# ndefilippis/SWRaytracing

Hardware: AMD Instinct MI355X
Metric: packet-steps/sec @ 512² field, 1e6 packets; 1/2/4/8-GPU scaling (higher is better)
Workload: dtype f64

## Files before the change

### swraytracing_amd/csrc/swrt_api.hip

```cpp
#include <hip/hip_runtime.h>
#include <hip/hip_ext.h>

#include <cmath>
#include <cstdlib>
#include <cstring>
#include <algorithm>
#include <climits>
#include <vector>

#include "../../include/swrt.h"
#include "swrt_bin.hpp"
#include "swrt_fft.hpp"
#include "swrt_kernels.hpp"
#include "swrt_tile.hpp"
#include "swrt_qg.hpp"
#include "swrt_ode23.hpp"
#include "swrt_xka.hpp"
#include "swrt_rsw.hpp"
#include "swrt_spectral.hpp"
#include "swrt_hazard.hpp"
#include "swrt_diag.hpp"
#include "swrt_raydiag.hpp"
#include "swrt_map.hpp"
#include "swrt_kmap.hpp"
// ... 2390 lines not shown
  if (which != 0 && which != 1) return fail(c, SWRT_ERR_ARG, "which must be 0 (current) or 1 (previous)");
  if (which == 1 && !q.has_prev) return fail(c, SWRT_ERR_STATE, "no previous qk before the first step");
  if (layer < 0 || layer >= q.g.nl) return fail(c, SWRT_ERR_ARG, "layer out of range");
  HIPCHK(c, hipSetDevice(c->device));
  const double2* src = (which == 0 ? q.qk.get() : q.qk_prev.get()) + layer * q.nhalf;
  const size_t bytes = sizeof(double2) * q.nhalf;
  if (dst_mode != 0 && dst_mode != 1 && dst_mode != 2) return fail(c, SWRT_ERR_ARG, "dst_mode must be 0, 1 or 2");
  if (dst_mode) {
    const hipStream_t ext = stream ? (hipStream_t)stream : on_qg.saved;
    if (dst_mode == 1) HIPCHK_RC(stream_order(c, ext, c->stream, 0));
    hipLaunchKernelGGL(export_half_kernel, dim3(nblocks(q.nhalf + 1, 256)), dim3(256), 0, c->stream, src, dst,
                       q.nhalf, tail);
    HIPCHK(c, hipGetLastError());
    HIPCHK_RC(stream_order(c, c->stream, ext, 1));
  } else {
    HIPCHK(c, hipMemcpyAsync(dst, src, bytes, hipMemcpyDeviceToHost, c->stream));
    HIPCHK(c, hipStreamSynchronize(c->stream));
    dst[2 * q.nhalf] = tail;
  }
  return SWRT_OK;
  GUARD_END(c)
}

int swrt_snapshot_qk(swrt_ctx* c, int slot, const double* qk, int src_on_device, void* stream, int64_t nx,
                     double L, double K_d2, double shear, double k_scale, int64_t ny_period) {
  int rc = check_slot_args(c, slot, nx);
  if (rc) return rc;
  GUARD_BEGIN_KEEP_CHAIN
  if (!qk) return fail(c, SWRT_ERR_ARG, "qk is NULL");
  if (!is_pow2(nx)) return fail(c, SWRT_ERR_ARG, "nx must be a power of two for the GPU FFT");
  if (!(L > 0)) return fail(c, SWRT_ERR_ARG, "L must be > 0");
  if (ny_period == 0) ny_period = nx;
  if (ny_period % nx) return fail(c, SWRT_ERR_ARG, "ny_period must be a multiple of nx");
  if (c->qg.init && c->qg.g.n != nx) return fail(c, SWRT_ERR_ARG, "nx differs from the QG state's");
  HIPCHK(c, hipSetDevice(c->device));
  const hipStream_t pk = c->stream;
  if (!c->xq.init && !c->qg.init && c->qg_sep) mark_slots_used(c, pk);
  c->xq.init = true;
  OnQGStream on_qg(c);
  const int n = (int)nx, kmax = n / 2 - 1;
  const int64_t nn = nx * nx, nhalf = (int64_t)(2 * kmax + 1) * (kmax + 1);
  if (c->xq.nx != nx) {
    HIPCHK(c, hipStreamSynchronize(c->stream));
    c->xq.nx = 0;
    HIPCHK(c, c->xq.Z.alloc(3 * nn));
    HIPCHK(c, c->xq.T.alloc(3 * nn));
    HIPCHK(c, c->xq.fk.alloc(nhalf));
    c->xq.nx = nx;
  }
  if ((rc = ensure_twiddles(c, n))) return rc;
  if ((rc = qg_slot_acquire(c, slot))) return rc;
  if ((rc = ensure_slot(c, slot, nx))) return rc;
  const hipStream_t ext = stream ? (hipStream_t)stream : pk;
  const double2* fk = (const double2*)qk;
  if (src_on_device) {
    HIPCHK_RC(stream_order(c, ext, c->stream, 0));
  } else {
    HIPCHK(c, hipMemcpyAsync(c->xq.fk.get(), qk, sizeof(double2) * nhalf, hipMemcpyHostToDevice, c->stream));
    HIPCHK(c, hipStreamSynchronize(c->stream));
    fk = c->xq.fk.get();
  }
  if ((rc = fields_from_halfplane(c, slot, fk, n, 1, K_d2, k_scale, shear, 0, c->xq.Z.get(), c->xq.T.get(), n / 2, 1)))
    return rc;
  if (src_on_device) HIPCHK_RC(stream_order(c, c->stream, ext, 1));
  Slot& s = c->slot[slot];
  s.L = L;
  s.ny_period = ny_period;
  return qg_slot_written(c, slot);
  GUARD_END(c)
}

int swrt_swap_slots(swrt_ctx* c, int a, int b) {
  if (!c) return SWRT_ERR_ARG;
  if (a < 0 || a >= SWRT_MAX_SLOTS || b < 0 || b >= SWRT_MAX_SLOTS) return fail(c, SWRT_ERR_ARG, "slot out of range");
  std::swap(c->slot[a], c->slot[b]);
  return SWRT_OK;
}


int swrt_ode23_f1(swrt_ctx* c, double t, double tmax, double f, double Cg, int nslots, double thr, double bump,
                  double* rh_raw_out) {
  if (!c) return SWRT_ERR_ARG;
  GUARD_BEGIN
  HIPCHK_RC(lost_check(c));
  SlotUse slot_use(c, false, kSlots01);
  int rc;
  if ((rc = ode23_f1_queue(c, t, tmax, f, Cg, nslots, thr, bump))) return rc;
  return read_max(c, rh_raw_out);
  GUARD_END(c)
}

int swrt_ode23_attempt(swrt_ctx* c, double t, double h, double tnew, double tmax, double f, double Cg,
                       int nslots, double thr, double bump, double* err_raw_out) {
  if (!c) return SWRT_ERR_ARG;
  GUARD_BEGIN
  HIPCHK_RC(lost_check(c));
  SlotUse slot_use(c, false, kSlots01);
  HIPCHK(c, hipSetDevice(c->device));
  return ode23_attempt(c, t, h, tnew, tmax, f, Cg, nslots, thr, bump, c->o23.dense, err_raw_out);
  GUARD_END(c)
}

int swrt_ode23_accept(swrt_ctx* c) {
  if (!c) return SWRT_ERR_ARG;
  c->s0_dirty = true;
  if (c->in_hook) return fail(c, SWRT_ERR_STATE, "this call may touch the packets: not allowed inside an ode23 hook");
  HIPCHK_RC(lost_check(c));
  HIPCHK_RC(chain_drop(c));
  if (!c->o23.ynx) return fail(c, SWRT_ERR_STATE, "no ode23 step attempted");
  ode23_accept_sets(c);
  return SWRT_OK;
}

int swrt_ode23_set_dense(swrt_ctx* c, int on) {
  if (!c) return SWRT_ERR_ARG;
  c->s0_dirty = true;
  if (on != 0 && on != 1) return fail(c, SWRT_ERR_ARG, "dense must be 0 or 1");
  c->o23.dense = on != 0;
  c->o23.dense_ready = false;
  return SWRT_OK;
}

int swrt_ode23_ntrp(swrt_ctx* c, double t, double tnew, const double* tout, int64_t nout) {
  if (!c) return SWRT_ERR_ARG;
  HOOK_REFUSE
  GUARD_BEGIN_KEEP_CHAIN
  HIPCHK_RC(lost_check(c));
  if (nout < 0) return fail(c, SWRT_ERR_ARG, "nout < 0");
  if (nout > 0 && !tout) return fail(c, SWRT_ERR_ARG, "NULL buffer");
  if (!c->o23.dense_ready)
    return fail(c, SWRT_ERR_STATE,
                "ode23 ntrp: no dense attempt in the stage buffers (swrt_ode23_set_dense 1, then "
                "swrt_ode23_attempt; valid until swrt_ode23_accept or any other packet call)");
  const double tdir = std::copysign(1.0, tnew - t);
  if (!(tnew != t) || !std::isfinite(t) || !std::isfinite(tnew)) return fail(c, SWRT_ERR_ARG, "ode23 ntrp: empty step");
  for (int64_t i = 0; i < nout; ++i)
    if (!(tdir * (tout[i] - t) >= 0 && tdir * (tnew - tout[i]) >= 0))
      return fail(c, SWRT_ERR_ARG, "ode23 ntrp: an output time lies outside the step");
  if (nout == 0) return SWRT_OK;
  HIPCHK(c, hipSetDevice(c->device));
  HIPCHK_RC(ensure_history(c, nout));
  return ode23_ntrp_queue(c, t, tnew, tout, nout);
  GUARD_END(c)
}

int swrt_ode23_run_at(swrt_ctx* c, const double* tspan, int64_t nt, double tmax, double f, double Cg, int nslots,
                      double rtol, double atol, double bump, double* ts_out, int64_t ts_cap, int64_t* nts_out,
                      int64_t* stats3_out) {
  if (!c) return SWRT_ERR_ARG;
  if (!tspan) return fail(c, SWRT_ERR_ARG, "tspan is NULL");
  if (nt < 2) return fail(c, SWRT_ERR_ARG, "tspan needs at least two times");
  if (!ts_out || ts_cap < 1 || !nts_out) return fail(c, SWRT_ERR_ARG, "ts_out / ts_cap / nts_out");
  for (int64_t i = 0; i < nt; ++i)
    if (!std::isfinite(tspan[i])) return fail(c, SWRT_ERR_ARG, "tspan must be finite");
  {
    const double tdir = std::copysign(1.0, tspan[nt - 1] - tspan[0]);
    for (int64_t i = 1; i < nt; ++i)
      if (!(tdir * (tspan[i] - tspan[i - 1]) > 0))
        return fail(c, SWRT_ERR_ARG, "tspan must be strictly increasing or strictly decreasing");
  }
  GUARD_BEGIN
  HIPCHK_RC(lost_check(c));
  SlotUse slot_use(c, false, kSlots01);
  O23Stats st;
  int64_t nts = 0;
  const int rc = ode23_run_at(c, tspan, nt, tmax, f, Cg, nslots, rtol, atol, bump, ts_out, ts_cap, &nts, &st);
  if (rc == kO23BelowHmin) return fail(c, SWRT_ERR_STATE, "ode23: step size below hmin");
  if (rc) return rc;
  *nts_out = nts;
  if (stats3_out) {
    stats3_out[0] = st.steps;
    stats3_out[1] = st.failed;
    stats3_out[2] = st.attempts;
  }
  c->o23.last = st;
  return SWRT_OK;
  GUARD_END(c)
}

int swrt_ode23_chain_next(swrt_ctx* c, int slot_a, int slot_b) {
  if (!c) return SWRT_ERR_ARG;
  if (slot_a < 0 || slot_a >= SWRT_MAX_SLOTS || slot_b < 0 || slot_b >= SWRT_MAX_SLOTS || slot_a == slot_b)
    return fail(c, SWRT_ERR_ARG, "chain slots out of range or equal");
  c->o23.chain.want = true;
  c->o23.chain.sa = slot_a;
  c->o23.chain.sb = slot_b;
  return SWRT_OK;
}

int swrt_ode23_run(swrt_ctx* c, double t0, double tfinal, double tmax, double f, double Cg, int nslots,
                   double rtol, double atol, double bump, double* ts_out, int64_t ts_cap, int64_t* nts_out,
                   int64_t* stats3_out) {
  return swrt_ode23_run_hooked(c, t0, tfinal, tmax, f, Cg, nslots, rtol, atol, bump, ts_out, ts_cap, nts_out,
                               stats3_out, nullptr, nullptr);
}

int swrt_ode23_run_hooked(swrt_ctx* c, double t0, double tfinal, double tmax, double f, double Cg, int nslots,
                          double rtol, double atol, double bump, double* ts_out, int64_t ts_cap, int64_t* nts_out,
                          int64_t* stats3_out, void (*hook)(void*), void* hook_user) {
  return swrt_ode23_run_sharded(c, t0, tfinal, tmax, f, Cg, nslots, rtol, atol, bump, ts_out, ts_cap, nts_out,
                                stats3_out, hook, hook_user, nullptr, nullptr);
}

int swrt_ode23_run_sharded(swrt_ctx* c, double t0, double tfinal, double tmax, double f, double Cg, int nslots,
                           double rtol, double atol, double bump, double* ts_out, int64_t ts_cap, int64_t* nts_out,
                           int64_t* stats3_out, void (*hook)(void*), void* hook_user,
                           int (*reduce)(double*, void*), void* reduce_user) {
  if (!c) return SWRT_ERR_ARG;
  if (!ts_out || ts_cap < 1 || !nts_out) return fail(c, SWRT_ERR_ARG, "ts_out / ts_cap / nts_out");
  if (c->in_hook) return fail(c, SWRT_ERR_STATE, "an ode23 hook may not start another ode23 call");
  GUARD_BEGIN_KEEP_CHAIN
  HIPCHK_RC(lost_check(c));
  SlotUse slot_use(c, false, kSlots01);
  const double rtol_c = std::max(rtol, 100 * 2.220446049250313e-16);
  const double thr = atol / rtol_c;
  const double htspan = std::fabs(tfinal - t0);
  const double hmax = 0.1 * htspan;
  const double c0 = 0.8 * std::pow(rtol_c, 1.0 / 3.0);
  int rc;
  int sl_f1;
  Ode23State::O23Chain& ch = c->o23.chain;
  const bool first_cand = ch.first_q && same_bits(t0, 0.0) && same_bits(tfinal, ch.tfinal) &&
                          same_bits(tmax, ch.tmax) && same_bits(rtol, ch.rtol);
  ch.first_q = false;
  const bool taken = ode23_chain_take(c, t0, tmax, f, Cg, nslots, thr, bump);
  if (!(taken && first_cand)) HIPCHK_RC(chain_join(c));
  if (taken) {
    sl_f1 = ch.dmax_slot;
    ++ch.taken;
  } else {
    if ((rc = ode23_f1_queue(c, t0, tmax, f, Cg, nslots, thr, bump))) return rc;
    sl_f1 = c->o23.dmax_cur;
    c->o23.dmax_cur = (sl_f1 + 1) % 3;
  }
  Ode23Args base;
  if ((rc = ode23_prepare(c, nslots, base, tmax, f, Cg, thr, bump))) return rc;
  const bool dev_first = !reduce && tile_binned(c);
  const bool split = ode23_split_ok(c);
  const bool first_chained = taken && first_cand && dev_first && split == ch.split;
  uint64_t ticket = 0;
  if (first_chained) {
    ticket = ch.first_ticket;
    c->o23.chain_b = false;
    if (split) c->b_pending = 1;
    ++ch.first_taken;
  } else {
    HIPCHK_RC(chain_join(c));
    if (dev_first) {
      HIPCHK_RC(ode23_first_step_queue(c, sl_f1, c0, hmax, htspan, t0, tfinal, split, &ticket));
    } else {
      HIPCHK(c, hipMemcpyAsync(c->o23.hmax.get() + sl_f1, c->o23.dmax.get() + sl_f1, sizeof(unsigned long long),
                               hipMemcpyDeviceToHost, c->stream));
      HIPCHK(c, hipEventRecord(c->o23.ev[sl_f1].get(), c->stream));
    }
    if (split) {
      HIPCHK(c, hipStreamWaitEvent(c->sx[0].get(), c->o23.ev[sl_f1].get(), 0));
      if (c->hz.on) {
        c->hz.record(c->o23.ev[sl_f1].get(), 0);
        c->hz.wait(1, c->o23.ev[sl_f1].get());
      }
      c->b_pending = 1;
    }
  }
  DeviceExec ex(c, base, split, dev_first, sl_f1, hook, hook_user, reduce, reduce_user);
  ex.expect_ticket(ticket);
  if (first_chained)
    ex.adopt_first(ch.first_slot, ch.first_wg);
  else if (dev_first && (rc = ex.queue_first()))
    return rc;
  O23Stats st;
  int64_t nts = 0;
  rc = ode23_control(ex, t0, tfinal, rtol, atol, ts_out, ts_cap, &nts, &st);
  if (rc == kO23BelowHmin) return fail(c, SWRT_ERR_STATE, "ode23: step size below hmin");
  if (rc) return rc;
  if ((rc = ode23_chain_queue(c, tmax, f, Cg, nslots, thr, bump, rtol, reduce == nullptr))) return rc;
  *nts_out = nts;
  if (stats3_out) {
    stats3_out[0] = st.steps;
    stats3_out[1] = st.failed;
    stats3_out[2] = st.attempts;
  }
  c->o23.last = st;
  c->o23.first_taken += st.first_taken;
  c->o23.guesses_taken += st.guesses_taken[0] + st.guesses_taken[1] + st.guesses_taken[2];
  c->o23.split_runs += split ? 1 : 0;
  return SWRT_OK;
  GUARD_END(c)
}

#ifdef SWRT_PHASE_TIMING
int swrt_debug_phases(unsigned long long* out, int ntiles, int clear) {
  if (hipDeviceSynchronize() != hipSuccess) return SWRT_ERR_HIP;
  const size_t bytes = (size_t)ntiles * 8 * sizeof(unsigned long long);
  if (out && hipMemcpyFromSymbol(out, HIP_SYMBOL(swrt::swrt_phase_dbg), bytes, 0, hipMemcpyDeviceToHost) != hipSuccess)
    return SWRT_ERR_HIP;
  if (clear) {
    static unsigned long long zeros[16384 * 8];
    if (hipMemcpyToSymbol(HIP_SYMBOL(swrt::swrt_phase_dbg), zeros, sizeof(zeros), 0,
                          hipMemcpyHostToDevice) != hipSuccess)
      return SWRT_ERR_HIP;
  }
  return SWRT_OK;
}
#endif

}
```

### swraytracing_amd/csrc/swrt_tile.hpp

```cpp
#pragma once
#include <hip/hip_runtime.h>
#include <stdint.h>

#include "swrt_kernels.hpp"

namespace swrt {

struct TileArgs {
  StepArgs s;
  double* x_out;
  double* k_out;
  int* perm_out;
  const int* starts;
  const int* order;
  int ntx;
  int* next_keys;
  int* next_counts;
  int sort_cells;
  const int* src;
  double sort_lead;
  TileShare sh;
  int ivmode;
  int nint;
  const double* ivn[kMaxIntervals + 1];
  double ivdt[kMaxIntervals];
  StageArgs stg;
};

__device__ __forceinline__ auto tile_args_again() {
  auto* p = (const __attribute__((address_space(4))) TileArgs*)__builtin_amdgcn_kernarg_segment_ptr();
  asm volatile("" : "+s"(p));
  return p;
}

__device__ __forceinline__ const double* iv_nodes(const TileArgs& ta, int i) {
  const double* p = ta.ivn[0];
#pragma unroll
  for (int j = 1; j <= kMaxIntervals; ++j)
    if (i == j) p = ta.ivn[j];
  return p;
}
__device__ __forceinline__ double iv_dt(const TileArgs& ta, int i) {
  double d = ta.ivdt[0];
#pragma unroll
  for (int j = 1; j < kMaxIntervals; ++j)
    if (i == j) d = ta.ivdt[j];
  return d;
}

__device__ __forceinline__ int wg_work_range(const int* starts, const int* order, int64_t n, const TileShare& sh,
                                             int& pbeg, int& pend) {
  int tile = share_slot(sh, (int)blockIdx.x);
  if (order != nullptr) tile = order[tile];
  const int nn = (int)n;
  pbeg = min(max(starts[tile], 0), nn);
  pend = min(max(starts[tile + 1], pbeg), nn);
  return tile;
}
__device__ __forceinline__ int wg_work_range(const int* starts, int64_t n, int& pbeg, int& pend) {
  TileShare sh;
  sh.ntiles = (int)gridDim.x;
  return wg_work_range(starts, nullptr, n, sh, pbeg, pend);
}

__device__ __forceinline__ int wg_work(const TileArgs& ta, int& pbeg, int& pend) {
  return wg_work_range(ta.starts, ta.order, ta.s.n, ta.sh, pbeg, pend);
}

__device__ __forceinline__ int ring_diff(int a, int b, int n) {
  int d = a - b;
  if (d >= n / 2) d -= n;
  if (d < -n / 2) d += n;
  return d;
}

__device__ __forceinline__ int b128_lane_rank(int lane) {
  const int h = lane & 32, t = lane & 31;
  int k;
  if (t < 4) k = t;
  else if (t < 12) k = 16 + (t - 4);
  else if (t < 16) k = 4 + (t - 12);
  else if (t < 20) k = 24 + (t - 16);
  else if (t < 28) k = 8 + (t - 20);
  else k = t;
  return h + k;
}

template <bool TWO>
struct Tap6 {
  double2 a0, a1, a2, b0, b1, b2;
};
template <bool TWO, int WN>
__device__ __forceinline__ void tap6_read(const double2* p, int e, Tap6<TWO>& t) {
  t.a0 = p[0 * WN + e];
  t.a1 = p[1 * WN + e];
  t.a2 = p[2 * WN + e];
  if constexpr (TWO) {
    t.b0 = p[3 * WN + e];
    t.b1 = p[4 * WN + e];
    t.b2 = p[5 * WN + e];
  }
}
template <bool TWO, int W, int WN>
__device__ __forceinline__ void gather6_lds(const double2* lds, int node0, const Stencil& s,
                                            double o0[kRec], double o1[kRec]) {
#pragma unroll
  for (int f = 0; f < kRec; ++f) { o0[f] = -0.0; o1[f] = -0.0; }
  const double2* p = lds + node0;
  double wx[kNT], wy[kNT];
#pragma unroll
  for (int q = 0; q < kNT; ++q) {
    wx[q] = s.wx[q];
    wy[q] = s.wy[q];
    asm volatile("" : "+v"(wx[q]));
    asm volatile("" : "+v"(wy[q]));
  }
  if constexpr (TWO) {
#pragma unroll
    for (int i = 0; i < kNT; ++i) {
#pragma unroll
      for (int j = 0; j < kNT; ++j) {
        const int e = i * W + j;
        const double wij = wx[i] * wy[j];
        const double2 a0 = p[0 * WN + e], a1 = p[1 * WN + e], a2 = p[2 * WN + e];
        o0[0] = o0[0] + wij * a0.x; o0[1] = o0[1] + wij * a0.y;
        o0[2] = o0[2] + wij * a1.x; o0[3] = o0[3] + wij * a1.y;
        o0[4] = o0[4] + wij * a2.x; o0[5] = o0[5] + wij * a2.y;
        const double2 b0 = p[3 * WN + e], b1 = p[4 * WN + e], b2 = p[5 * WN + e];
        o1[0] = o1[0] + wij * b0.x; o1[1] = o1[1] + wij * b0.y;
        o1[2] = o1[2] + wij * b1.x; o1[3] = o1[3] + wij * b1.y;
        o1[4] = o1[4] + wij * b2.x; o1[5] = o1[5] + wij * b2.y;
      }
    }
    return;
  }
  Tap6<TWO> cur, nxt;
  tap6_read<TWO, WN>(p, 0, cur);
#pragma unroll
  for (int t = 0; t < kNT * kNT; ++t) {
    const int i = t / kNT, j = t % kNT;
    if (t + 1 < kNT * kNT) tap6_read<TWO, WN>(p, ((t + 1) / kNT) * W + (t + 1) % kNT, nxt);
    if constexpr (!TWO) __builtin_amdgcn_sched_barrier(0);
    const double wij = wx[i] * wy[j];
    o0[0] = o0[0] + wij * cur.a0.x; o0[1] = o0[1] + wij * cur.a0.y;
    o0[2] = o0[2] + wij * cur.a1.x; o0[3] = o0[3] + wij * cur.a1.y;
    o0[4] = o0[4] + wij * cur.a2.x; o0[5] = o0[5] + wij * cur.a2.y;
    if constexpr (TWO) {
      o1[0] = o1[0] + wij * cur.b0.x; o1[1] = o1[1] + wij * cur.b0.y;
      o1[2] = o1[2] + wij * cur.b1.x; o1[3] = o1[3] + wij * cur.b1.y;
      o1[4] = o1[4] + wij * cur.b2.x; o1[5] = o1[5] + wij * cur.b2.y;
    }
    if constexpr (!TWO) __builtin_amdgcn_sched_barrier(0);
    if (t + 1 < kNT * kNT) cur = nxt;
  }
}

template <bool TWO>
struct Tap5 {
  double2 a0, a1, c, b0, b1;
};
template <bool TWO, int WN>
__device__ __forceinline__ void tap5_read(const double2* p, int e, Tap5<TWO>& t) {
  t.a0 = p[0 * WN + e];
  t.a1 = p[1 * WN + e];
  if constexpr (TWO) {
    t.c = p[2 * WN + e];
    t.b0 = p[3 * WN + e];
    t.b1 = p[4 * WN + e];
  } else {
    t.c.x = reinterpret_cast<const double*>(p + 2 * WN + e)[0];
  }
}
template <bool TWO, int W, int WN, bool FMA = false, int PF = 1>
__device__ __forceinline__ void gather5_lds(const double2* lds, int node0, const Stencil& s,
                                            double o0[kRec], double o1[kRec]) {
  static_assert(PF >= 1 && PF <= 4, "prefetch depth");
  constexpr int NTAP = kNT * kNT;
#pragma unroll
  for (int f = 0; f < 5; ++f) { o0[f] = -0.0; o1[f] = -0.0; }
  const double2* p = lds + node0;
  double wx[kNT], wy[kNT];
#pragma unroll
  for (int q = 0; q < kNT; ++q) {
    wx[q] = s.wx[q];
    wy[q] = s.wy[q];
    asm volatile("" : "+v"(wx[q]));
    asm volatile("" : "+v"(wy[q]));
  }
  Tap5<TWO> ring[PF + 1];
#pragma unroll
  for (int t = 0; t < PF; ++t) tap5_read<TWO, WN>(p, (t / kNT) * W + t % kNT, ring[t]);
#pragma unroll
  for (int t = 0; t < NTAP; ++t) {
    const int i = t / kNT, j = t % kNT;
    if (t + PF < NTAP) tap5_read<TWO, WN>(p, ((t + PF) / kNT) * W + (t + PF) % kNT, ring[(t + PF) % (PF + 1)]);
    __builtin_amdgcn_sched_barrier(0);
    const Tap5<TWO>& cur = ring[t % (PF + 1)];
    const double wij = wx[i] * wy[j];
    o0[0] = madd<FMA>(o0[0], wij, cur.a0.x); o0[1] = madd<FMA>(o0[1], wij, cur.a0.y);
    o0[2] = madd<FMA>(o0[2], wij, cur.a1.x); o0[3] = madd<FMA>(o0[3], wij, cur.a1.y);
    o0[4] = madd<FMA>(o0[4], wij, cur.c.x);
    if constexpr (TWO) {
      o1[0] = madd<FMA>(o1[0], wij, cur.b0.x); o1[1] = madd<FMA>(o1[1], wij, cur.b0.y);
      o1[2] = madd<FMA>(o1[2], wij, cur.b1.x); o1[3] = madd<FMA>(o1[3], wij, cur.b1.y);
      o1[4] = madd<FMA>(o1[4], wij, cur.c.y);
    }
    __builtin_amdgcn_sched_barrier(0);
  }
  o0[5] = -o0[2];
  o1[5] = -o1[2];
}

template <bool TWO, int W, int WN>
__device__ __forceinline__ void gather2_lds(const double2* lds, int node0, const Stencil& s, double o0[2],
                                            double o1[2]) {
  constexpr int NTAP = kNT * kNT;
  o0[0] = o0[1] = -0.0;
  o1[0] = o1[1] = -0.0;
  const double2* p = lds + node0;
  double wx[kNT], wy[kNT];
#pragma unroll
  for (int q = 0; q < kNT; ++q) {
    wx[q] = s.wx[q];
    wy[q] = s.wy[q];
    asm volatile("" : "+v"(wx[q]));
    asm volatile("" : "+v"(wy[q]));
  }
  double2 ra[2], rb[2];
  ra[0] = p[0];
  if constexpr (TWO) rb[0] = p[3 * WN];
#pragma unroll
  for (int t = 0; t < NTAP; ++t) {
    const int i = t / kNT, j = t % kNT;
    if (t + 1 < NTAP) {
      const int e = ((t + 1) / kNT) * W + (t + 1) % kNT;
      ra[(t + 1) & 1] = p[e];
      if constexpr (TWO) rb[(t + 1) & 1] = p[3 * WN + e];
    }
    __builtin_amdgcn_sched_barrier(0);
    const double wij = wx[i] * wy[j];
    o0[0] = o0[0] + wij * ra[t & 1].x; o0[1] = o0[1] + wij * ra[t & 1].y;
    if constexpr (TWO) {
      o1[0] = o1[0] + wij * rb[t & 1].x; o1[1] = o1[1] + wij * rb[t & 1].y;
    }
    __builtin_amdgcn_sched_barrier(0);
  }
}

template <bool TWO, int WN, bool V5>
__device__ __forceinline__ void stage_record(const double2* s0, const double2* s1, int d, double2* win) {
  if constexpr (V5 && TWO) {
    const double2 a0 = s0[0], a1 = s0[1], a2 = s0[2], b0 = s1[0], b1 = s1[1], b2 = s1[2];
    win[0 * WN + d] = a0;
    win[1 * WN + d] = a1;
    win[2 * WN + d] = make_double2(a2.x, b2.x);
    win[3 * WN + d] = b0;
    win[4 * WN + d] = b1;
  } else if constexpr (TWO) {
    const double2 a0 = s0[0], a1 = s0[1], a2 = s0[2], b0 = s1[0], b1 = s1[1], b2 = s1[2];
    win[0 * WN + d] = a0;
    win[1 * WN + d] = a1;
    win[2 * WN + d] = a2;
    win[3 * WN + d] = b0;
    win[4 * WN + d] = b1;
    win[5 * WN + d] = b2;
  } else {
    const double2 a0 = s0[0], a1 = s0[1], a2 = s0[2];
    win[0 * WN + d] = a0;
    win[1 * WN + d] = a1;
    win[2 * WN + d] = a2;
  }
}
template <bool TWO, int T, int M, int NT, int WS = T + 5 + 2 * M, bool V5 = false>
__device__ __forceinline__ void stage_window_regs(const FieldView& f0, const FieldView& f1, int ox, int oy,
                                                  double2* win) {
  constexpr int W = T + 5 + 2 * M;
  constexpr int WN = W * WS;
  constexpr int CW = W <= 32 ? 32 : (W <= 64 ? 64 : 128);
  constexpr int RP = NT / CW;
  static_assert(W <= CW && NT % CW == 0, "window rows per workgroup pass");
  const int nx = f0.nx, npad = f0.npad;
  const int wj = (int)threadIdx.x % CW;
  int wi = (int)threadIdx.x / CW;
  if (wj >= W) return;
  const char* n0 = reinterpret_cast<const char*>(f0.nodes);
  const char* n1 = reinterpret_cast<const char*>(f1.nodes);
  constexpr unsigned kRecBytes = kRec * sizeof(double);
  if (nx >= W && (uint64_t)npad * (uint64_t)npad * kRecBytes < (1ull << 32)) {
    int gy = oy - M - 2 + wj;
    gy += gy < 0 ? nx : 0;
    gy -= gy >= nx ? nx : 0;
    const unsigned col = (unsigned)(gy + kPadLo) * kRecBytes;
    const unsigned rowb = (unsigned)npad * kRecBytes;
    for (int d = wi * WS + wj; wi < W; wi += RP, d += RP * WS) {
      int gx = ox - M - 2 + wi;
      gx += gx < 0 ? nx : 0;
      gx -= gx >= nx ? nx : 0;
      const unsigned off = (unsigned)(gx + kPadLo) * rowb + col;
      stage_record<TWO, WN, V5>(reinterpret_cast<const double2*>(n0 + off),
                                reinterpret_cast<const double2*>(n1 + off), d, win);
    }
  } else {
    int gy = (oy - M - 2 + wj) % nx; gy += gy < 0 ? nx : 0;
    for (; wi < W; wi += RP) {
      int gx = (ox - M - 2 + wi) % nx; gx += gx < 0 ? nx : 0;
      const size_t off = ((size_t)(gx + kPadLo) * npad + (gy + kPadLo)) * kRecBytes;
      stage_record<TWO, WN, V5>(reinterpret_cast<const double2*>(n0 + off),
                                reinterpret_cast<const double2*>(n1 + off), wi * WS + wj, win);
    }
  }
}

#ifdef SWRT_PHASE_TIMING
__device__ unsigned long long swrt_phase_dbg[16384 * 8];
#define SWRT_STAMP(slot)                                                            \
  do {                                                                              \
    if (tid == 0) swrt_phase_dbg[blockIdx.x * 8 + (slot)] = __builtin_amdgcn_s_memrealtime(); \
  } while (0)
#else
#define SWRT_STAMP(slot) \
  do {                   \
  } while (0)
#endif

template <int T, int NT, int NB>
__device__ __forceinline__ void sort_batch_by_cell(int b0, int nb, bool first_batch, int tile, int* hist,
                                                   int* kr, int* order) {
  const auto* g = tile_args_again();
  int tid = threadIdx.x;
  asm volatile("" : "+v"(tid));
  const int nx = g->s.f0.nx;
  const int tx = (int)((unsigned)tile / (unsigned)g->ntx), ty = tile - tx * g->ntx;
  const int ox = tx * T, oy = ty * T;
  const int64_t n = g->s.n;
  const double* xin = g->s.x;
  const double* kin = g->s.k;
  const int* srcp = g->src;
  const double sort_lead = g->sort_lead, gH = g->s.gH, f2 = g->s.f2, inv_dx = g->s.f0.inv_dx;
  for (int h = tid; h < NB; h += NT) hist[h] = 0;
  __syncthreads();
  if (first_batch) SWRT_STAMP(1);
  for (int i = tid; i < nb; i += NT) {
    const int64_t p = srcp ? srcp[b0 + i] : b0 + i;
    double xs = xin[p], ys = xin[n + p];
    if (sort_lead != 0.0) {
      const double kx = kin[p], ky = kin[n + p];
      const double s = sort_lead * gH / sqrt(f2 + gH * (kx * kx + ky * ky));
      xs += s * kx;
      ys += s * ky;
    }
    const int ic = fast_cell(xs, inv_dx, nx);
    const int jc = fast_cell(ys, inv_dx, nx);
    const int dx_ = min(max(ring_diff(ic, ox, nx), 0), T - 1);
    const int dy_ = min(max(ring_diff(jc, oy, nx), 0), T - 1);
    int key;
    if constexpr (T == 16) {
      key = (dx_ >= 0 && dx_ < T && dy_ >= 0 && dy_ < T)
                ? ((dy_ & 1) | ((dx_ & 1) << 1) | ((dy_ & 2) << 1) | ((dx_ & 2) << 2) |
                   ((dy_ & 4) << 2) | ((dx_ & 4) << 3) | ((dy_ & 8) << 3) | ((dx_ & 8) << 4))
                : T * T;
    } else {
      key = 0;
#pragma unroll
      for (int b = 0; (1 << b) < T; ++b) key |= (((dy_ >> b) & 1) << (2 * b)) | (((dx_ >> b) & 1) << (2 * b + 1));
    }
    const int r = atomicAdd(&hist[key], 1);
    kr[i] = (key << 16) | r;
  }
  __syncthreads();
  if (tid < 64) {
    constexpr int PER = (NB + 63) / 64;
    int loc[PER];
    int sum = 0;
#pragma unroll
    for (int q = 0; q < PER; ++q) {
      const int h = tid * PER + q;
      loc[q] = h < NB ? hist[h] : 0;
      sum += loc[q];
    }
    int incl = sum;
#pragma unroll
    for (int off = 1; off < 64; off <<= 1) {
      const int v = __shfl_up(incl, off, 64);
      if (tid >= off) incl += v;
    }
    int run = incl - sum;
#pragma unroll
    for (int q = 0; q < PER; ++q) {
      const int h = tid * PER + q;
      if (h < NB) hist[h] = run;
      run += loc[q];
    }
  }
  __syncthreads();
  for (int i = tid; i < nb; i += NT) {
    const int v = kr[i];
    order[hist[v >> 16] + (v & 0xffff)] = srcp ? srcp[b0 + i] : b0 + i;
  }
  __syncthreads();
}

template <bool TWO, int T, int M, int WS, int WNP, bool V5, bool UV>
__device__ __forceinline__ void tile_flow_at(const double2* win, const FieldView& f0, const double* n0,
                                             const double* n1, int oxm, int oym, double x, double y, double bump,
                                             double sgd, int j, double I[kRec]) {
  const int nx = f0.nx;
  Stencil sc;
  stencil_at(f0, x, y, bump, sc);
  const int d0 = sc.ic - oxm, d1 = sc.jc - oym;
  const unsigned ux = min((unsigned)d0, (unsigned)(d0 + nx)), uy = min((unsigned)d1, (unsigned)(d1 + nx));
  const bool inwin = max(ux, uy) < (unsigned)(T + 2 * M);
  double J[kRec];
  if constexpr (UV) {
    if (inwin)
      gather2_lds<TWO, WS, WNP>(win, (int)(ux * WS + uy), sc, I, J);
    else
      gather2<TWO, true>(n0, n1, f0.npad, sc, I, J);
  } else {
    if (inwin) {
      if constexpr (V5)
        gather5_lds<TWO, WS, WNP>(win, (int)(ux * WS + uy), sc, I, J);
      else
        gather6_lds<TWO, WS, WNP>(win, (int)(ux * WS + uy), sc, I, J);
    } else {
      gather6_lean<TWO>(n0, n1, f0.npad, sc, I, J);
    }
  }
  if constexpr (TWO) {
    const auto* g = tile_args_again();
    const double dalpha = g->s.dalpha;
    const double alpha = (g->s.alpha0 + sgd * dalpha) + g->stg.off[j] * dalpha;
    const double oma = 1 - alpha;
#pragma unroll
    for (int q = 0; q < (UV ? 2 : (V5 ? 5 : kRec)); ++q) I[q] = oma * I[q] + alpha * J[q];
    if constexpr (V5 && !UV) I[5] = -I[2];
  }
}

__device__ __forceinline__ double tile_stage_h(int j, double dt) {
  const auto* g = tile_args_again();
  return g->stg.w[j] * dt;
}

#ifndef SWRT_TILE_MIN_WAVES
#define SWRT_TILE_MIN_WAVES 4
#endif

template <bool TWO, int T, int M, int NT, bool V5 = false, bool FMA = false, int PF = 1,
          int MINW = SWRT_TILE_MIN_WAVES, bool HIST = true, bool MULTI = true, bool STG = false>
__global__ void __launch_bounds__(NT, MINW) tile_leapfrog_kernel(TileArgs ta) {
  static_assert(!FMA || V5, "the FMA gather exists for the five-sum window only");
  static_assert(!STG || (HIST && MULTI && !FMA && PF == 1), "the staged step exists for the general form only");
  constexpr int W = T + 5 + 2 * M;
  constexpr int WS = W + ((12 - W % 16) + 16) % 16;
  constexpr int WNP = W * WS;
  constexpr int NCH = TWO ? (V5 ? 5 : 6) : 3;
  constexpr int NB = T * T + 1;
  constexpr int MAXB = 2 * NT;
  __shared__ double2 win[NCH * WNP];
  __shared__ int hist[NB];
  __shared__ int kr[MAXB];
  __shared__ int order[MAXB];
  __shared__ int nbr[9];
#ifdef SWRT_PHASE_TIMING
  __shared__ int nfall;
  __shared__ unsigned simds;
#endif

  const StepArgs& a = ta.s;
  const int tid = threadIdx.x;
  int pbeg, pend;
  const int tile = min(max(__builtin_amdgcn_readfirstlane(wg_work(ta, pbeg, pend)), 0), ta.ntx * ta.ntx - 1);
  pbeg = __builtin_amdgcn_readfirstlane(pbeg);
  pend = __builtin_amdgcn_readfirstlane(pend);
  const int nx = a.f0.nx, npad = a.f0.npad;
  int ox, oy;
  {
    const int tx = (int)((unsigned)tile / (unsigned)ta.ntx), ty = tile - tx * ta.ntx;
    ox = tx * T;
    oy = ty * T;
  }
  int oxm = ox - M, oym = oy - M;
  if (nx >= M) {
    oxm += oxm < 0 ? nx : 0;
    oym += oym < 0 ? nx : 0;
  } else {
    oxm = (oxm % nx + nx) % nx;
    oym = (oym % nx + nx) % nx;
  }
  if (tid < 9) nbr[tid] = tid == 4 ? pend - pbeg : 0;
#ifdef SWRT_PHASE_TIMING
  if (tid == 0) nfall = 0;
  if (tid == 0) simds = 0;
#endif
  SWRT_STAMP(0);
#ifdef SWRT_PHASE_TIMING
  if (tid == 0) {
    unsigned hw, xcc;
    asm volatile("s_getreg_b32 %0, hwreg(HW_REG_HW_ID)" : "=s"(hw));
    asm volatile("s_getreg_b32 %0, hwreg(HW_REG_XCC_ID)" : "=s"(xcc));
    swrt_phase_dbg[blockIdx.x * 8 + 7] = ((unsigned long long)xcc << 32) | hw;
    swrt_phase_dbg[blockIdx.x * 8 + 6] = (unsigned long long)(pend - pbeg);
  }
  __syncthreads();
  if ((tid & 63) == 0) {
    unsigned hw;
    asm volatile("s_getreg_b32 %0, hwreg(HW_REG_HW_ID)" : "=s"(hw));
    atomicOr(&simds, ((hw >> 4) & 3u) << (2 * (tid >> 6)));
  }
  __syncthreads();
  if (tid == 0) swrt_phase_dbg[blockIdx.x * 8 + 6] |= (unsigned long long)simds << 32;
#endif

  const unsigned lane_rank = (unsigned)b128_lane_rank(tid & 63);
  const int wave0 = __builtin_amdgcn_readfirstlane(tid & ~63);
  const bool ivmode = MULTI && ta.ivmode;
  const int nint = ivmode ? ta.nint : 1;
  for (int ivl = 0; ivl < nint; ++ivl) {
  FieldView fa = a.f0, fb = a.f1;
  if (ivmode) {
    fa.nodes = iv_nodes(ta, ivl);
    fb.nodes = iv_nodes(ta, ivl + 1);
  }
  const double dt = ivmode ? iv_dt(ta, ivl) : a.dt;
  const double half = ivmode ? 0.5 * dt : a.half;
  const bool first = !MULTI || ivl == 0;
  const int sortc = first ? ta.sort_cells : 0;
  const bool last = !MULTI || ivl == nint - 1;
  const int64_t sbase = a.s0 + (int64_t)ivl * a.nsteps;
  if (!first) __syncthreads();

  stage_window_regs<TWO, T, M, NT, WS, V5>(fa, fb, ox, oy, win);
  if (!sortc) {
    __syncthreads();
    SWRT_STAMP(1);
  }
  const int bstep = sortc ? MAXB : max(pend - pbeg, 1);
  for (int b0 = pbeg; b0 < pend; b0 += bstep) {
    const int nb = min(bstep, pend - b0);
    if (sortc) sort_batch_by_cell<T, NT, NB>(b0, nb, b0 == pbeg, tile, hist, kr, order);
    if (b0 == pbeg) SWRT_STAMP(2);

    for (int r0 = wave0; r0 < nb; r0 += NT) {
      const int r = r0 + (int)lane_rank;
      if (r >= nb) continue;
      const int64_t slot0 = (int64_t)b0 + r0;
      double x0, y0, k0, l0;
      int orig;
      {
        const auto* g = tile_args_again();
        const int64_t n = g->s.n;
        const double* xi = first ? g->s.x : g->x_out;
        const double* ki = first ? g->s.k : g->k_out;
        const int* pi_ = first ? g->s.perm : g->perm_out;
        if (sortc) {
          const int64_t pi = order[r];
          x0 = xi[pi]; y0 = xi[n + pi];
          k0 = ki[pi]; l0 = ki[n + pi];
          orig = pi_[pi];
        } else {
          const double* xr = xi + slot0;
          const double* kr_ = ki + slot0;
          x0 = xr[lane_rank]; y0 = (xr + n)[lane_rank];
          k0 = kr_[lane_rank]; l0 = (kr_ + n)[lane_rank];
          orig = (pi_ + slot0)[lane_rank];
        }
      }
      double hcx, hcy;
      drift_inc(k0, l0, a.f2, a.gH, half, a.fastdisp, hcx, hcy);
      double sgd = (double)(ivmode ? (int64_t)0 : sbase);
      double qx = 0.0, qy = 0.0;
      if constexpr (STG) drift_quot(k0, l0, a.f2, a.gH, a.fastdisp, qx, qy);
      for (int st = 0; st < a.nsteps; ++st) {
        if constexpr (STG) {
          const auto* gk = tile_args_again();
          const int nstages = gk->stg.nstages;
          const bool midpoint = gk->stg.kick != 0;
          const int nit = midpoint ? gk->stg.iters : 0;
          for (int j = 0; j < nstages; ++j) {
            double x1, y1;
            {
              const double hh = 0.5 * tile_stage_h(j, dt);
              x1 = x0 + hh * qx;
              y1 = y0 + hh * qy;
            }
            double xm = x1, ym = y1;
            double I[kRec];
            for (int it = 0; it < nit; ++it) {
              tile_flow_at<TWO, T, M, WS, WNP, V5, true>(win, a.f0, fa.nodes, fb.nodes, oxm, oym, xm, ym, a.bump,
                                                         sgd, j, I);
              const double hh = 0.5 * tile_stage_h(j, dt);
              xm = x1 + hh * I[0];
              ym = y1 + hh * I[1];
            }
            tile_flow_at<TWO, T, M, WS, WNP, V5, false>(win, a.f0, fa.nodes, fb.nodes, oxm, oym, xm, ym, a.bump,
                                                        sgd, j, I);
            const double h = tile_stage_h(j, dt);
            const double hh = 0.5 * h;
            const double x2 = x1 + h * I[0];
            const double y2 = y1 + h * I[1];
            double k2, l2;
            kick_k(midpoint, h, hh, I, k0, l0, k2, l2);
            drift_quot(k2, l2, a.f2, a.gH, a.fastdisp, qx, qy);
            x0 = x2 + hh * qx;
            y0 = y2 + hh * qy;
            k0 = k2;
            l0 = l2;
          }
          sgd = sgd + 1.0;
        } else {
        const double alpha = a.alpha0 + sgd * a.dalpha;
        sgd = sgd + 1.0;
        const double x1 = x0 + hcx;
        const double y1 = y0 + hcy;
        Stencil sc;
        stencil_at(a.f0, x1, y1, a.bump, sc);
        const int d0 = sc.ic - oxm, d1 = sc.jc - oym;
        const unsigned ux = min((unsigned)d0, (unsigned)(d0 + nx)), uy = min((unsigned)d1, (unsigned)(d1 + nx));
        double I[kRec], J[kRec];
        const bool inwin = max(ux, uy) < (unsigned)(T + 2 * M);
#ifdef SWRT_PHASE_TIMING
        if (!inwin) atomicAdd(&nfall, 1);
#endif
        if (inwin) {
          if constexpr (V5)
            gather5_lds<TWO, WS, WNP, FMA, PF>(win, (int)(ux * WS + uy), sc, I, J);
          else
            gather6_lds<TWO, WS, WNP>(win, (int)(ux * WS + uy), sc, I, J);
        } else {
          if constexpr (MULTI) {
            gather6_lean<TWO, FMA>(fa.nodes, fb.nodes, npad, sc, I, J);
          } else {
            const auto* g = tile_args_again();
            gather6_lean<TWO, FMA>(g->s.f0.nodes, g->s.f1.nodes, g->s.f0.npad, sc, I, J);
          }
        }
        if constexpr (TWO) {
          const double oma = 1 - alpha;
#pragma unroll
          for (int q = 0; q < (V5 ? 5 : kRec); ++q) I[q] = madd<FMA>(oma * I[q], alpha, J[q]);
          if constexpr (V5) I[5] = -I[2];
        }
        const double x2 = x1 + dt * I[0];
        const double y2 = y1 + dt * I[1];
        const double k2 = k0 - dt * (I[2] * k0 + I[4] * l0);
        const double l2 = l0 - dt * (I[3] * k0 + I[5] * l0);
        drift_inc(k2, l2, a.f2, a.gH, half, a.fastdisp, hcx, hcy);
        x0 = x2 + hcx;
        y0 = y2 + hcy;
        k0 = k2;
        l0 = l2;
        }
        if constexpr (HIST) {
          const int64_t sg = sbase + st;
          if (a.hist_x != nullptr && ((sg + 1) % a.save_every) == 0) {
            const int64_t fr = a.frame0 + (sg + 1) / a.save_every - 1;
            double* hx = a.hist_x + fr * 2 * a.n;
            double* hk = a.hist_k + fr * 2 * a.n;
            hx[orig] = x0; hx[a.n + orig] = y0;
            hk[orig] = k0; hk[a.n + orig] = l0;
          }
        }
      }
      const auto* g = tile_args_again();
      const int64_t n = g->s.n;
      double* xw = g->x_out + slot0;
      double* kw = g->k_out + slot0;
      xw[lane_rank] = x0; (xw + n)[lane_rank] = y0;
      kw[lane_rank] = k0; (kw + n)[lane_rank] = l0;
      (g->perm_out + slot0)[lane_rank] = orig;
      int* nkeys = g->next_keys;
      if (last && nkeys != nullptr) {
        const int64_t po = slot0 + lane_rank;
        const int nxk = g->s.f0.nx;
        const int ic = fast_cell(x0, a.f0.inv_dx, nxk);
        const int jc = fast_cell(y0, a.f0.inv_dx, nxk);
        const int ntx_ = g->ntx;
        const int tx = (int)((unsigned)tile / (unsigned)ntx_), ty = tile - tx * ntx_;
        const int ntx2 = ic / T, nty2 = jc / T;
        nkeys[po] = ntx2 * ntx_ + nty2;
        const int ddx = ring_diff(ntx2, tx, ntx_), ddy = ring_diff(nty2, ty, ntx_);
        if (ddx != 0 || ddy != 0) {
          atomicAdd(&nbr[4], -1);
          if (ddx >= -1 && ddx <= 1 && ddy >= -1 && ddy <= 1)
            atomicAdd(&nbr[(ddx + 1) * 3 + (ddy + 1)], 1);
          else
            atomicAdd(&g->next_counts[ntx2 * ntx_ + nty2], 1);
        }
      }
    }
#ifdef SWRT_PHASE_TIMING
    __syncthreads();
#else
    if (sortc) __syncthreads();
#endif
    if (b0 == pbeg) SWRT_STAMP(3);
  }
  }
  const auto* g = tile_args_again();
  if (g->next_keys != nullptr) {
    __syncthreads();
    int t9 = tid;
    asm volatile("" : "+v"(t9));
    const int v = t9 < 9 ? nbr[t9] : 0;
    if (v != 0) {
      const int n_ = g->ntx;
      const int tx = (int)((unsigned)tile / (unsigned)n_), ty = tile - tx * n_;
      const int gx = ((tx + t9 / 3 - 1) % n_ + n_) % n_, gy = ((ty + t9 % 3 - 1) % n_ + n_) % n_;
      atomicAdd(&g->next_counts[gx * n_ + gy], v);
    }
  }
  SWRT_STAMP(4);
#ifdef SWRT_PHASE_TIMING
  __syncthreads();
  if (tid == 0) swrt_phase_dbg[blockIdx.x * 8 + 5] = (unsigned long long)nfall;
#endif
}

}
```

Before: 26.67 billion.

## Distribute packet chunks to waves dynamically via LDS atomic counter

Replaces the static per-wave stride over packets in the tile leapfrog kernel with dynamic work claiming. Each wave grabs 64-packet chunks from a shared-memory atomic counter, so waves that finish early pick up more work and load imbalance within a workgroup shrinks. The counter is never reset between sort batches or intervals; the code instead subtracts an interval offset, which is fragile, and each chunk now costs an LDS atomic plus a readfirstlane. It also adds per-wave end-time debug stamps under the phase-timing build flag.

```diff
diff --git a/swraytracing_amd/csrc/swrt_api.hip b/swraytracing_amd/csrc/swrt_api.hip
--- a/swraytracing_amd/csrc/swrt_api.hip
+++ b/swraytracing_amd/csrc/swrt_api.hip
@@ -2716,6 +2716,20 @@
   }
   return SWRT_OK;
 }
+
+int swrt_debug_wave_ends(unsigned long long* out, int ntiles, int clear) {
+  if (hipDeviceSynchronize() != hipSuccess) return SWRT_ERR_HIP;
+  const size_t bytes = (size_t)ntiles * 8 * sizeof(unsigned long long);
+  if (out && hipMemcpyFromSymbol(out, HIP_SYMBOL(swrt::swrt_wave_dbg), bytes, 0, hipMemcpyDeviceToHost) != hipSuccess)
+    return SWRT_ERR_HIP;
+  if (clear) {
+    static unsigned long long zeros[16384 * 8];
+    if (hipMemcpyToSymbol(HIP_SYMBOL(swrt::swrt_wave_dbg), zeros, sizeof(zeros), 0,
+                          hipMemcpyHostToDevice) != hipSuccess)
+      return SWRT_ERR_HIP;
+  }
+  return SWRT_OK;
+}
 #endif
 
 }
diff --git a/swraytracing_amd/csrc/swrt_tile.hpp b/swraytracing_amd/csrc/swrt_tile.hpp
--- a/swraytracing_amd/csrc/swrt_tile.hpp
+++ b/swraytracing_amd/csrc/swrt_tile.hpp
@@ -313,6 +313,7 @@
 
 #ifdef SWRT_PHASE_TIMING
 __device__ unsigned long long swrt_phase_dbg[16384 * 8];
+__device__ unsigned long long swrt_wave_dbg[16384 * 8];
 #define SWRT_STAMP(slot)                                                            \
   do {                                                                              \
     if (tid == 0) swrt_phase_dbg[blockIdx.x * 8 + (slot)] = __builtin_amdgcn_s_memrealtime(); \
@@ -322,6 +323,21 @@
   do {                   \
   } while (0)
 #endif
+
+__device__ __forceinline__ unsigned lane_id_here() {
+  unsigned z = 0;
+  asm volatile("" : "+v"(z));
+  return __builtin_amdgcn_mbcnt_hi(~0u, __builtin_amdgcn_mbcnt_lo(~0u, z));
+}
+
+__device__ __forceinline__ int claim_chunk(int* next) {
+  auto* p = (__attribute__((address_space(3))) int*)next;
+  int inc = 64;
+  asm volatile("" : "+v"(p), "+v"(inc));
+  int c = 0;
+  if (lane_id_here() == 0) c = __hip_atomic_fetch_add(p, inc, __ATOMIC_RELAXED, __HIP_MEMORY_SCOPE_WORKGROUP);
+  return __builtin_amdgcn_readfirstlane(c);
+}
 
 template <int T, int NT, int NB>
 __device__ __forceinline__ void sort_batch_by_cell(int b0, int nb, bool first_batch, int tile, int* hist,
@@ -462,6 +478,7 @@
   __shared__ int kr[MAXB];
   __shared__ int order[MAXB];
   __shared__ int nbr[9];
+  __shared__ int claimed;
 #ifdef SWRT_PHASE_TIMING
   __shared__ int nfall;
   __shared__ unsigned simds;
@@ -489,6 +506,7 @@
     oym = (oym % nx + nx) % nx;
   }
   if (tid < 9) nbr[tid] = tid == 4 ? pend - pbeg : 0;
+  if (tid == 9) claimed = NT;
 #ifdef SWRT_PHASE_TIMING
   if (tid == 0) nfall = 0;
   if (tid == 0) simds = 0;
@@ -514,6 +532,9 @@
 
   const unsigned lane_rank = (unsigned)b128_lane_rank(tid & 63);
   const int wave0 = __builtin_amdgcn_readfirstlane(tid & ~63);
+#ifdef SWRT_PHASE_TIMING
+  int wave_chunks = 0;
+#endif
   const bool ivmode = MULTI && ta.ivmode;
   const int nint = ivmode ? ta.nint : 1;
   for (int ivl = 0; ivl < nint; ++ivl) {
@@ -535,16 +556,23 @@
     __syncthreads();
     SWRT_STAMP(1);
   }
-  const int bstep = sortc ? MAXB : max(pend - pbeg, 1);
-  for (int b0 = pbeg; b0 < pend; b0 += bstep) {
-    const int nb = min(bstep, pend - b0);
-    if (sortc) sort_batch_by_cell<T, NT, NB>(b0, nb, b0 == pbeg, tile, hist, kr, order);
-    if (b0 == pbeg) SWRT_STAMP(2);
-
-    for (int r0 = wave0; r0 < nb; r0 += NT) {
-      const int r = r0 + (int)lane_rank;
+  const int npk = pend - pbeg;
+  const int bstep = sortc ? MAXB : max(npk, 1);
+  const int tot64 = (npk + 63) & ~63;
+  for (int bq = 0; bq < npk; bq += bstep) {
+    const int b0 = pbeg + bq;
+    const int nb = min(bstep, npk - bq);
+    if (sortc) sort_batch_by_cell<T, NT, NB>(b0, nb, bq == 0, tile, hist, kr, order);
+    if (bq == 0) SWRT_STAMP(2);
+
+    const int qend = bq + nb;
+    for (int q0 = bq + wave0; q0 < qend; q0 = claim_chunk(&claimed) - (MULTI ? ivl * tot64 : 0)) {
+#ifdef SWRT_PHASE_TIMING
+      ++wave_chunks;
+#endif
+      const int r = (q0 - bq) + (int)lane_rank;
       if (r >= nb) continue;
-      const int64_t slot0 = (int64_t)b0 + r0;
+      const int64_t slot0 = (int64_t)pbeg + q0;
       double x0, y0, k0, l0;
       int orig;
       {
@@ -553,7 +581,7 @@
         const double* xi = first ? g->s.x : g->x_out;
         const double* ki = first ? g->s.k : g->k_out;
         const int* pi_ = first ? g->s.perm : g->perm_out;
-        if (sortc) {
+        if (first && g->sort_cells) {
           const int64_t pi = order[r];
           x0 = xi[pi]; y0 = xi[n + pi];
           k0 = ki[pi]; l0 = ki[n + pi];
@@ -690,11 +718,13 @@
       }
     }
 #ifdef SWRT_PHASE_TIMING
+    if ((tid & 63) == 0)
+      swrt_wave_dbg[blockIdx.x * 8 + (tid >> 6)] = (__builtin_amdgcn_s_memrealtime() << 8) | (unsigned)wave_chunks;
     __syncthreads();
 #else
     if (sortc) __syncthreads();
 #endif
-    if (b0 == pbeg) SWRT_STAMP(3);
+    if (bq == 0) SWRT_STAMP(3);
   }
   }
   const auto* g = tile_args_again();
```

Result: no change. 26.77 billion, median of 6 (+0.4%).
